# HanielUlises/GCN-GrabCut

Measured on AMD Instinct MI355X. Metric: images/sec end-to-end mask (DUTS-shape batch), higher is better.
Workload: dtype f32

## Files before the change

### gcn-grabcut_amd/csrc/ggc_ccl.h

```cpp
#pragma once
#include <hip/hip_runtime.h>
#include <cstdint>

namespace ggc {

__device__ __forceinline__ int ccl_find(const int32_t* parent, int i) {
    int p = __hip_atomic_load(&parent[i], __ATOMIC_RELAXED, __HIP_MEMORY_SCOPE_AGENT);
    while (p != i) { i = p; p = __hip_atomic_load(&parent[i], __ATOMIC_RELAXED, __HIP_MEMORY_SCOPE_AGENT); }
    return i;
}
__device__ __forceinline__ void ccl_union(int32_t* parent, int a, int b) {
    for (;;) {
        a = ccl_find(parent, a); b = ccl_find(parent, b);
        if (a == b) return;
        if (a < b) { const int t = a; a = b; b = t; }
        const int old = atomicMin(&parent[a], b);
        if (old == a) return;
        a = old;
    }
}

__host__ __device__ inline int ccl_run_start_lane(unsigned long long starts, int lane) {
    const unsigned long long below = starts & ((2ull << lane) - 1ull);
#if defined(__HIP_DEVICE_COMPILE__)
    return 63 - __clzll((long long)below);
#else
    return 63 - __builtin_clzll(below);
#endif
}
__host__ __device__ inline int ccl_run_length(unsigned long long starts, unsigned long long vmask, int lane) {
    const unsigned long long stop = (starts | ~vmask) >> lane >> 1;
#if defined(__HIP_DEVICE_COMPILE__)
    return stop ? __ffsll((long long)stop) : 64 - lane;
#else
    return stop ? __builtin_ffsll((long long)stop) : 64 - lane;
#endif
}

__device__ __forceinline__ int ccl_run_first(bool on, bool same_left, int p) {
    const int lane = threadIdx.x & 63;
    const unsigned long long starts = __ballot(on && (!same_left || lane == 0));
    return p - (lane - ccl_run_start_lane(starts, lane));
}

template <int CONN, class Joined>
__device__ __forceinline__ void ccl_merge_pixel(int32_t* par, int p, int x, bool has_up, int W, size_t flat, Joined joined) {
    static_assert(CONN == 4 || CONN == 8, "4 or 8 neighbours");
    const bool left = x > 0 && joined(p - 1);
    if (left && (flat & 63) == 0) ccl_union(par, p, p - 1);
    if (!has_up) return;
    if constexpr (CONN == 4) {
        if (joined(p - W) && !(left && joined(p - W - 1))) ccl_union(par, p, p - W);
    } else {
        const bool up = joined(p - W);
        const bool ul = x > 0 && joined(p - W - 1), ur = x + 1 < W && joined(p - W + 1);
        if (left) {
            if (ur && !up) ccl_union(par, p, p - W + 1);
        } else if (up) {
            ccl_union(par, p, p - W);
        } else {
            if (ul) ccl_union(par, p, p - W - 1);
            if (ur) ccl_union(par, p, p - W + 1);
        }
    }
}

__device__ __forceinline__ int ccl_compress(int32_t* par, int p) { const int r = ccl_find(par, p); par[p] = r; return r; }
__device__ __forceinline__ void ccl_count_runs(bool valid, bool same_left, unsigned long long vmask, int32_t* counts, size_t cell) {
    const int lane = threadIdx.x & 63;
    const unsigned long long starts = __ballot(valid && (!same_left || lane == 0));
    if (valid && ((starts >> lane) & 1ull)) atomicAdd(&counts[cell], ccl_run_length(starts, vmask, lane));
}

__host__ __device__ inline unsigned long long ccl_best_key(int area, int root) {
    return ((unsigned long long)(unsigned)area << 32) | (unsigned long long)(0xFFFFFFFFu - (unsigned)root);
}
__host__ __device__ inline int ccl_best_root(unsigned long long key) { return (int)(0xFFFFFFFFu - (unsigned)(key & 0xFFFFFFFFull)); }

}
```

### gcn-grabcut_amd/csrc/ggc_context.hip

```cpp
#include "ggc_internal.h"
#include <algorithm>
#include <cstdarg>
#include <cstdlib>
#include <mutex>

static thread_local std::string g_create_err;

namespace ggc {

const Knobs& knobs() {
    static const Knobs k = [] {
        auto num = [](const char* name, int dflt, int lo) { const char* e = std::getenv(name); return e ? std::max(lo, std::atoi(e)) : dflt; };
        Knobs k;
        k.mf_trace = std::getenv("GGC_MF_TRACE") != nullptr;
        k.mf_warm = num("GGC_MF_WARM", 1, 0);
        k.mf_async_push_active = num("GGC_MF_ASYNC_PUSH_ACTIVE", 10000, 0);
        k.mf_async_tile = num("GGC_MF_ASYNC_TILE", 8, 8);
        k.mf_async_hops = num("GGC_MF_ASYNC_HOPS", 24, 1);
        k.mf_async_sweeps = num("GGC_MF_ASYNC_SWEEPS", 12, 1);
        k.mf_dense_launches = num("GGC_MF_DENSE_LAUNCHES", 12, 1);
        k.mf_dense_launches0 = num("GGC_MF_DENSE_LAUNCHES0", 8, 1);
        k.mf_dense_sweeps = num("GGC_MF_DENSE_SWEEPS", 8, 1);
        k.mf_relax_dense = num("GGC_MF_RELAX_DENSE", 3, 1);
        k.mf_partial_rounds = std::min(64, num("GGC_MF_PARTIAL_ROUNDS", 3, 0));
        k.agg_direct = num("GGC_AGG_DIRECT", 0, 0);
        k.slic_seq_connectivity = num("GGC_SLIC_SEQ_CONNECTIVITY", 0, 0);
        k.matte_eval_levels = num("GGC_MATTE_EVAL_LEVELS", 0, 0);
        if (k.matte_eval_levels > 10 || (k.matte_eval_levels && 10 % k.matte_eval_levels != 0)) k.matte_eval_levels = 0;
        k.graph_onchip = num("GGC_GRAPH_ONCHIP", 1, 0);
        k.graph_bands = num("GGC_GRAPH_BANDS", 0, 0);
        if (k.graph_bands > 8) k.graph_bands = 0;
        k.wand_seeds_per_pass = num("GGC_WAND_SEEDS_PER_PASS", 0, 0);
        if (k.wand_seeds_per_pass > 4096) k.wand_seeds_per_pass = 0;
        return k;
    }();
    return k;
}

int set_err(ggc_ctx* ctx, int code, const char* fmt, ...) {
    char buf[1024];
    va_list ap;
    va_start(ap, fmt);
    vsnprintf(buf, sizeof(buf), fmt, ap);
    va_end(ap);
    if (ctx) ctx->err = buf; else g_create_err = buf;
    return code;
}

void* scratch(ggc_ctx* ctx, int slot, size_t bytes) {
    Buf& b = ctx->slots[slot];
    if (bytes == 0) bytes = 16;
    if (b.bytes >= bytes) return b.p;
    if (b.p) {
        if (hipFree(b.p) != hipSuccess) { set_err(ctx, GGC_E_DEVICE, "hipFree failed"); return nullptr; }
        b.p = nullptr; b.bytes = 0;
    }
    size_t want = bytes + bytes / 4;
    want = (want + 255) & ~size_t(255);
    void* p = nullptr;
    if (hipMalloc(&p, want) != hipSuccess) {
        set_err(ctx, GGC_E_OOM, "hipMalloc(%zu) failed for scratch slot %d", want, slot);
        return nullptr;
    }
    b.p = p; b.bytes = want;
    return p;
}

int read_i32(ggc_ctx* ctx, hipStream_t st, const int32_t* dev, int n, std::vector<int32_t>& host) {
    host.resize(n);
    if (ctx->h_pinned && n <= ggc_ctx::H_PINNED_INTS) {
        GGC_HIP(ctx, hipMemcpyAsync(ctx->h_pinned, dev, sizeof(int32_t) * n, hipMemcpyDeviceToHost, st));
        GGC_HIP(ctx, hipStreamSynchronize(st));
        std::copy(ctx->h_pinned, ctx->h_pinned + n, host.begin());
        return GGC_OK;
    }
    GGC_HIP(ctx, hipMemcpyAsync(host.data(), dev, sizeof(int32_t) * n, hipMemcpyDeviceToHost, st));
    GGC_HIP(ctx, hipStreamSynchronize(st));
    return GGC_OK;
}

int check_offsets(ggc_ctx* ctx, const int32_t* off, int n, const char* name, const char* unit, int min_step) {
    GGC_REQUIRE(ctx, off[0] == 0, GGC_E_INVALID_ARG, "%s[0] = %d, expected 0", name, off[0]);
    for (int i = 0; i < n; ++i)
        GGC_REQUIRE(ctx, (int64_t)off[i + 1] - off[i] >= min_step, GGC_E_INVALID_ARG,
                    "%s decreases at %s %d, or steps by less than %d (%d -> %d)", name, unit, i, min_step, off[i], off[i + 1]);
    return GGC_OK;
}

int read_offsets(ggc_ctx* ctx, hipStream_t st, const int32_t* dev, int n, const char* name, const char* unit, int min_step,
                 std::vector<int32_t>& host) {
    const int rc = read_i32(ctx, st, dev, n + 1, host);
    return rc ? rc : check_offsets(ctx, host.data(), n, name, unit, min_step);
}

}

extern "C" {

int ggc_version(void) { return GGC_VERSION; }

int ggc_ctx_create(int device_id, ggc_ctx** out) {
    if (!out) return ggc::set_err(nullptr, GGC_E_INVALID_ARG, "out is NULL");
    *out = nullptr;
    int n = 0;
    hipError_t e = hipGetDeviceCount(&n);
    if (e != hipSuccess || n <= 0)
        return ggc::set_err(nullptr, GGC_E_DEVICE, "no HIP device available (%s)",
                            e == hipSuccess ? "count=0" : hipGetErrorString(e));
    if (device_id < 0 || device_id >= n)
// ... 78 lines not shown
```

### gcn-grabcut_amd/csrc/ggc_internal.h

```cpp
#pragma once
#include <hip/hip_runtime.h>
#include <cstdint>
#include <cstdio>
#include <atomic>
#include <cstring>
#include <map>
#include <string>
#include <type_traits>
#include <vector>
#include "../../include/ggc.h"
#include "../../include/ggc_fmath.h"

namespace ggc {

constexpr int WAVE = 64;

enum Slot : int {
    S_CSR_ROWPTR = 0, S_CSR_COL, S_CSR_EID, S_CSR_CURSOR, S_CSR_SCAN, S_DIS, S_BATCH, S_AGG_PACK,
    S_STATES, S_GATE, S_XW, S_AGG, S_SCORE, S_GVEC, S_HJK,
    S_PRE_A, S_PRE_B, S_PRE_C, S_PRE_D,
    S_SLIC_IMG, S_SLIC_TMP, S_SLIC_CENTERS, S_SLIC_DIST, S_SLIC_LABELS, S_SLIC_AUX,
    S_SLIC_AUX2, S_SLIC_AUX3, S_SLIC_AUX4, S_SLIC_MINMAX,
    S_G_STATS, S_G_FEAT, S_G_PAIRS, S_G_PAIRCNT, S_G_NL, S_G_LISTS, S_G_EDGE_DST,
    S_G_EDGE_ATTR, S_G_PTR, S_G_PRIOR, S_G_AUX, S_G_AUX2, S_G_AUX3, S_G_X,
// ... 1 lines not shown
    S_GC_A, S_GC_B, S_GC_C, S_GC_D, S_GC_E, S_GC_F, S_GC_G, S_GC_H, S_GC_I, S_GC_J,
    S_GC_K, S_GC_L, S_GC_M,
    S_CC_A, S_CC_B, S_CC_C,
    S_MISC_A, S_MISC_B,
    S_CLICK,
    S_MATTE, S_MATTE_MEAN, S_CFMATTE,
    S_FOREGROUND, S_FOREGROUND_VEC,
    S_MATTE_EVAL,
    S_FULLCUT,
    S_GEODESIC,
    S_STROKES,
    S_POLYGONS,
    S_SCISSORS,
    S_OUTLINE, S_OUTLINE_LIST,
    S_DIST, S_DIST_TMP,
    S_WAND,
    S_COUNT
};

struct Buf {
    void*  p = nullptr;
    size_t bytes = 0;
};

struct WeightSet {
    int D = 0;
    int Dt = 0;
    int n_layers = 0;
    int Q = 0, C = 0;
    int heads = 0;
    std::map<std::string, std::vector<float>> host;
    std::map<std::string, Buf> dev;
    bool dev_ok = false;
};

struct GraphState {
    int B = 0, H = 0, W = 0;
    int64_t n_total = 0, e_total = 0;
    std::vector<int64_t> node_ptr, edge_ptr;
    std::vector<int64_t> pair_ptr;
    int64_t max_pairs = 0;
    int n_max = 0;
    const int32_t* n_nodes_dev = nullptr;
    bool valid = false;
};

}

namespace ggc {
struct ProfRec { const char* name; hipEvent_t a, b; };
}

struct ggc_ctx {
    int device = 0;
    std::string err;
    int prof_on = 0;
    double prof_overhead_ms = 0.0;
    std::vector<ggc::ProfRec> prof;
    std::vector<hipEvent_t> prof_pool;
    ggc::Buf slots[ggc::S_COUNT];
    ggc::WeightSet resgcn, gcnnet, gat;
    ggc::GraphState graph;
    int n_cu = 256;
    float prior_two_ce2 = (float)(2 * 0.45 * 0.45), prior_two_cs2 = (float)(2 * 0.40 * 0.40);
    int32_t* h_pinned = nullptr;
    static constexpr int H_PINNED_INTS = 4096;
};

namespace ggc {

struct Knobs {
    int mf_trace;
    int mf_warm;
    int mf_async_push_active;
    int mf_async_tile;
    int mf_async_hops;
    int mf_async_sweeps;
    int mf_dense_launches0, mf_dense_launches;
    int mf_dense_sweeps;
    int mf_relax_dense;
    int mf_partial_rounds;
    int agg_direct;
    int slic_seq_connectivity;
    int matte_eval_levels;
    int graph_onchip;
    int graph_bands;
    int wand_seeds_per_pass;
};
const Knobs& knobs();

int set_err(ggc_ctx* ctx, int code, const char* fmt, ...);
int read_i32(ggc_ctx* ctx, hipStream_t st, const int32_t* dev, int n, std::vector<int32_t>& host);
int read_offsets(ggc_ctx* ctx, hipStream_t st, const int32_t* dev, int n, const char* name, const char* unit, int min_step,
                 std::vector<int32_t>& host);
int check_offsets(ggc_ctx* ctx, const int32_t* off, int n, const char* name, const char* unit, int min_step);
void* scratch(ggc_ctx* ctx, int slot, size_t bytes);
int build_csr(ggc_ctx* ctx, hipStream_t st, int N, int E, const int32_t* src, const int32_t* dst,
              int32_t* row_ptr, int32_t* col, int32_t* eid, int32_t* cursor, float* dis);

#define GGC_HIP(ctx, expr)                                                          \
    do {                                                                            \
        hipError_t _e = (expr);                                                     \
        if (_e != hipSuccess)                                                       \
            return ggc::set_err((ctx), GGC_E_DEVICE, "%s failed: %s (%s:%d)", #expr, \
                                hipGetErrorString(_e), __FILE__, __LINE__);          \
    } while (0)

#define GGC_LAUNCH_CHECK(ctx)                                                        \
    do {                                                                            \
        hipError_t _e = hipGetLastError();                                          \
        if (_e != hipSuccess)                                                       \
            return ggc::set_err((ctx), GGC_E_DEVICE, "kernel launch failed: %s (%s:%d)", \
                                hipGetErrorString(_e), __FILE__, __LINE__);          \
    } while (0)

#define GGC_REQUIRE(ctx, cond, code, ...)                      \
    do {                                                       \
        if (!(cond)) return ggc::set_err((ctx), (code), __VA_ARGS__); \
    } while (0)

template <typename T>
inline T* scratch_t(ggc_ctx* ctx, int slot, size_t count) {
    return reinterpret_cast<T*>(scratch(ctx, slot, count * sizeof(T)));
}

struct Carve {
    char* base = nullptr;
    size_t bytes = 0;
    template <typename T> T* take(size_t count) {
        T* p = base ? reinterpret_cast<T*>(base + bytes) : nullptr;
        bytes += (count * sizeof(T) + 255) & ~size_t(255);
        return p;
    }
};
template <typename Layout>
inline size_t carve_scratch(ggc_ctx* ctx, int slot, Layout&& layout) {
    Carve c;
    layout(c);
    c.base = static_cast<char*>(scratch(ctx, slot, c.bytes));
    if (!c.base) return 0;
    c.bytes = 0;
    layout(c);
    return c.bytes;
}

inline int cdiv(int64_t a, int64_t b) { return (int)((a + b - 1) / b); }

template <int... Ws, typename F>
bool with_width(int D, int& rc, F&& f) {
    return ((D == Ws && (rc = f(std::integral_constant<int, Ws>{}), true)) || ...);
}

struct DeviceOnce {
    std::atomic<unsigned long long> mask{0};
    bool need(int dev) const { return dev < 0 || dev >= 64 || !((mask.load(std::memory_order_acquire) >> dev) & 1ull); }
    void done(int dev) { if (dev >= 0 && dev < 64) mask.fetch_or(1ull << dev, std::memory_order_release); }
};

struct ProfScope {
    ggc_ctx* ctx; hipStream_t st; hipEvent_t b = nullptr;
    ProfScope(ggc_ctx* c, hipStream_t s, const char* name) : ctx(c), st(s) {
        if (!c->prof_on || (c->prof_on == 2 && std::strcmp(name, "gcn_aggregate") != 0)) return;
        hipEvent_t ev[2];
        for (int i = 0; i < 2; ++i) {
            if (!c->prof_pool.empty()) { ev[i] = c->prof_pool.back(); c->prof_pool.pop_back(); }
            else if (hipEventCreate(&ev[i]) != hipSuccess) return;
// ... 67 lines not shown
```

### gcn-grabcut_amd/csrc/ggc_slic.hip

```cpp
#include "ggc_internal.h"
#include "ggc_ccl.h"
#include "ggc_math.h"
#include <cmath>
#include <vector>

namespace ggc {

__global__ void k_minmax_init(int B, uint32_t* mm) {
    const int i = blockIdx.x * blockDim.x + threadIdx.x;
    if (i < B) { mm[2 * i] = 0xFFFFFFFFu; mm[2 * i + 1] = 0u; }
}

__global__ void __launch_bounds__(256) k_minmax(size_t n, const float* __restrict__ img, uint32_t* mm) {
    const float* im = img + (size_t)blockIdx.y * n;
    float lo = INFINITY, hi = -INFINITY;
    for (size_t i = (size_t)blockIdx.x * blockDim.x + threadIdx.x; i < n; i += (size_t)gridDim.x * blockDim.x) {
        const float v = im[i];
        lo = fminf(lo, v); hi = fmaxf(hi, v);
    }
    for (int o = 32; o > 0; o >>= 1) { lo = fminf(lo, __shfl_xor(lo, o, 64)); hi = fmaxf(hi, __shfl_xor(hi, o, 64)); }
    __shared__ float s_lo[4], s_hi[4];
    if ((threadIdx.x & 63) == 0) { s_lo[threadIdx.x >> 6] = lo; s_hi[threadIdx.x >> 6] = hi; }
    __syncthreads();
    if (threadIdx.x == 0) {
// ... 423 lines not shown
        same_left = (p % d.W) > 0 && pending[i - 1] && raw[i - 1] == raw[i];
        r = ccl_compress(parent + base, p);
    }
    ccl_count_runs(valid, same_left, __ballot(valid), csize, base + r);
}

__global__ void __launch_bounds__(256) k_cn_settle(CnDims d, uint8_t* __restrict__ pending, const int32_t* __restrict__ parent,
                                                   const int32_t* __restrict__ csize, int32_t* __restrict__ n_big) {
    const size_t i = (size_t)blockIdx.x * blockDim.x + threadIdx.x;
    if (i >= (size_t)d.B * d.P || !pending[i]) return;
    const size_t base = (i / d.P) * d.P;
    const int p = (int)(i - base), r = parent[i];
    if (csize[base + r] < d.max_size) pending[i] = 0;
    else if (p == r) atomicAdd(n_big, 1);
}

__global__ void __launch_bounds__(64) k_cn_carve(CnDims d, int tag, uint8_t* __restrict__ pending, const int32_t* __restrict__ parent,
                                                 int32_t* __restrict__ csize, int32_t* __restrict__ mark,
                                                 int32_t* __restrict__ queue, int32_t* __restrict__ qtop) {
    const size_t i = (size_t)blockIdx.x * blockDim.x + threadIdx.x;
    if (i >= (size_t)d.B * d.P) return;
    const int b = (int)(i / d.P);
    const size_t base = (size_t)b * d.P;
    const int r = (int)(i - base);
    if (!pending[i] || parent[i] != r || csize[i] < d.max_size) return;
    int32_t* q = queue + base + atomicAdd(&qtop[b], d.max_size);
    int size = 1, visited = 0;
    q[0] = r; mark[base + r] = tag;
    while (visited < size && size < d.max_size) {
        const int pc = q[visited];
        const int yc = pc / d.W, xc = pc - yc * d.W;
#pragma unroll
        for (int k = 0; k < 4; ++k) {
            const int xx = xc + (k == 0 ? 1 : k == 1 ? -1 : 0), yy = yc + (k == 2 ? 1 : k == 3 ? -1 : 0);
            if (xx < 0 || xx >= d.W || yy < 0 || yy >= d.H) continue;
            const int pp = yy * d.W + xx;
            if (pending[base + pp] && parent[base + pp] == r && mark[base + pp] != tag) {
                mark[base + pp] = tag;
                q[size++] = pp;
                if (size >= d.max_size) break;
            }
        }
        visited += 1;
    }
    for (int k = 0; k < size; ++k) pending[base + q[k]] = 0;
    csize[i] = size;
}

__global__ void __launch_bounds__(256) k_cn_kept(CnDims d, const int32_t* __restrict__ parent, const int32_t* __restrict__ csize,
                                                 int32_t* __restrict__ rank) {
    const size_t i = (size_t)blockIdx.x * blockDim.x + threadIdx.x;
    if (i >= (size_t)d.B * d.P) return;
    rank[i] = (parent[i] == (int)(i % d.P) && csize[i] >= d.min_size) ? 1 : 0;
}

__global__ void __launch_bounds__(1024) k_cn_scan(CnDims d, int32_t* __restrict__ rank, int32_t* __restrict__ n_nodes) {
    __shared__ int32_t wsum[16];
    __shared__ int32_t s_carry;
    const int b = blockIdx.x, tid = threadIdx.x, lane = tid & 63, wave = tid >> 6;
    int32_t* a = rank + (size_t)b * d.P;
    if (tid == 0) s_carry = 0;
    __syncthreads();
    for (int base = 0; base < d.P; base += 4096) {
        const int i0 = base + tid * 4;
        int32_t c[4], s = 0;
#pragma unroll
        for (int j = 0; j < 4; ++j) { c[j] = i0 + j < d.P ? a[i0 + j] : 0; s += c[j]; }
        int32_t incl = s;
        for (int o = 1; o < 64; o <<= 1) { const int32_t v = __shfl_up(incl, o, 64); if (lane >= o) incl += v; }
        if (lane == 63) wsum[wave] = incl;
        __syncthreads();
        int32_t run = s_carry + (incl - s), total = 0;
#pragma unroll
        for (int w = 0; w < 16; ++w) { if (w < wave) run += wsum[w]; total += wsum[w]; }
#pragma unroll
        for (int j = 0; j < 4; ++j) { if (i0 + j < d.P) a[i0 + j] = run; run += c[j]; }
        __syncthreads();
        if (tid == 0) s_carry += total;
        __syncthreads();
    }
    if (tid == 0) n_nodes[b] = s_carry > 0 ? s_carry : 1;
}

__global__ void __launch_bounds__(64) k_cn_small(CnDims d, int tag, const int32_t* __restrict__ parent,
                                                 const int32_t* __restrict__ csize, int32_t* __restrict__ mark,
                                                 int32_t* __restrict__ queue, int32_t* __restrict__ qtop,
                                                 int32_t* __restrict__ tgt) {
    const size_t i = (size_t)blockIdx.x * blockDim.x + threadIdx.x;
    if (i >= (size_t)d.B * d.P) return;
    const int b = (int)(i / d.P);
    const size_t base = (size_t)b * d.P;
    const int r = (int)(i - base);
    if (parent[i] != r || csize[i] >= d.min_size) return;
    const int n = csize[i];
    int32_t* q = queue + base + atomicAdd(&qtop[b], n);
    int size = 1, visited = 0, last = -1;
    q[0] = r; mark[base + r] = tag;
    while (visited < size) {
        const int pc = q[visited];
        const int yc = pc / d.W, xc = pc - yc * d.W;
#pragma unroll
        for (int k = 0; k < 4; ++k) {
            const int xx = xc + (k == 0 ? 1 : k == 1 ? -1 : 0), yy = yc + (k == 2 ? 1 : k == 3 ? -1 : 0);
            if (xx < 0 || xx >= d.W || yy < 0 || yy >= d.H) continue;
            const int pp = yy * d.W + xx;
            const int rp = parent[base + pp];
            if (rp == r) { if (mark[base + pp] != tag && size < n) { mark[base + pp] = tag; q[size++] = pp; } }
            else if (rp < r) last = rp;
        }
        visited += 1;
    }
    tgt[i] = last;
}

__global__ void __launch_bounds__(256) k_cn_write(CnDims d, const int32_t* __restrict__ parent, const int32_t* __restrict__ csize,
                                                  const int32_t* __restrict__ rank, const int32_t* __restrict__ tgt,
                                                  int32_t* __restrict__ out) {
    const size_t i = (size_t)blockIdx.x * blockDim.x + threadIdx.x;
    if (i >= (size_t)d.B * d.P) return;
    const size_t base = (i / d.P) * d.P;
    int r = parent[i];
    int lab = 0;
    for (;;) {
        if (csize[base + r] >= d.min_size) { lab = rank[base + r]; break; }
        const int t = tgt[base + r];
        if (t < 0) { lab = 0; break; }
        r = t;
    }
    out[i] = lab;
}


static double np_pairwise_sum(const double* a, int n) {
    if (n < 8) { double s = 0.0; for (int i = 0; i < n; ++i) s += a[i]; return s; }
    double r[8];
    for (int j = 0; j < 8; ++j) r[j] = a[j];
    int i;
    for (i = 8; i < n - (n % 8); i += 8) for (int j = 0; j < 8; ++j) r[j] += a[i + j];
    double res = ((r[0] + r[1]) + (r[2] + r[3])) + ((r[4] + r[5]) + (r[6] + r[7]));
    for (; i < n; ++i) res += a[i];
    return res;
}

struct Grid { int step_y, step_x, start_y, start_x, ny, nx, K; };
static Grid regular_grid(int H, int W, int n_points) {
    Grid g{};
    const double dims[3] = {1.0, (double)(H <= W ? H : W), (double)(H <= W ? W : H)};
    const double space = 1.0 * H * W;
    if (space <= (double)n_points) { g = {1, 1, 0, 0, H, W, H * W}; return g; }
    double st[3];
    for (int i = 0; i < 3; ++i) st[i] = std::pow(space / n_points, 1.0 / 3.0);
    if (dims[0] < st[0] || dims[1] < st[1] || dims[2] < st[2]) {
        for (int dim = 0; dim < 3; ++dim) {
            st[dim] = dims[dim];
            double sp = 1.0;
            for (int j = dim + 1; j < 3; ++j) sp *= dims[j];
            for (int j = dim + 1; j < 3; ++j) st[j] = std::pow(sp / n_points, 1.0 / (3 - dim - 1));
            if (dims[0] >= st[0] && dims[1] >= st[1] && dims[2] >= st[2]) break;
        }
    }
    int starts[3], steps[3];
    for (int i = 0; i < 3; ++i) { starts[i] = (int)std::floor(st[i] / 2.0); steps[i] = (int)std::rint(st[i]); }
    const int iy = (H <= W) ? 1 : 2, ix = (H <= W) ? 2 : 1;
    g.step_y = steps[iy]; g.start_y = starts[iy];
    g.step_x = steps[ix]; g.start_x = starts[ix];
    g.ny = std::max(0, (H - g.start_y + g.step_y - 1) / g.step_y);
    g.nx = std::max(0, (W - g.start_x + g.step_x - 1) / g.step_x);
    g.K = g.ny * g.nx;
    return g;
}

}

using namespace ggc;

static int enforce_connectivity(ggc_ctx* ctx, hipStream_t st, int B, int H, int W, const int32_t* raw, int min_size,
                                int max_size, int32_t* segments, int32_t* n_nodes) {
    const size_t P = (size_t)H * W;
    if (knobs().slic_seq_connectivity) {
        int32_t* queue = scratch_t<int32_t>(ctx, S_SLIC_AUX3, (size_t)B * (size_t)std::max(max_size, 1));
        if (!queue) return GGC_E_OOM;
        GGC_HIP(ctx, hipMemsetAsync(segments, 0xFF, sizeof(int32_t) * (size_t)B * P, st));
        ProfScope prof(ctx, st, "slic_connectivity");
        hipLaunchKernelGGL(k_connectivity_seq, dim3(B), dim3(64), 0, st, H, W, raw, min_size, max_size, queue, segments,
                           n_nodes);
        GGC_LAUNCH_CHECK(ctx);
        return GGC_OK;
    }
    {
        ProfScope prof(ctx, st, "slic_connectivity");
        const size_t BP = (size_t)B * P;
        const CnDims cd{B, H, W, (int)P, min_size, std::max(max_size, 1)};
        int32_t* work = scratch_t<int32_t>(ctx, S_SLIC_AUX3, BP * 6 + (size_t)B * (size_t)cd.max_size + 2 * (size_t)B + 16);
        uint8_t* pending = scratch_t<uint8_t>(ctx, S_SLIC_AUX4, BP);
        if (!work || !pending) return GGC_E_OOM;
        int32_t *parent = work, *csize = work + BP, *rank = work + 2 * BP, *tgt = work + 3 * BP, *mark = work + 4 * BP;
        int32_t* queue = work + 5 * BP;
        int32_t* qtop = work + 6 * BP + (size_t)B * cd.max_size;
        int32_t* n_big = qtop + B;
        GGC_HIP(ctx, hipMemsetAsync(pending, 1, BP, st));
        GGC_HIP(ctx, hipMemsetAsync(mark, 0, sizeof(int32_t) * BP, st));
        const dim3 g1(cdiv(BP, 256)), g2(cdiv(W, 64), cdiv(H, 4), B), g64(cdiv(BP, 64));
        for (int round = 0; round < 4096; ++round) {
            GGC_HIP(ctx, hipMemsetAsync(qtop, 0, sizeof(int32_t) * (B + 1), st));
            hipLaunchKernelGGL(k_cn_reset, g1, dim3(256), 0, st, cd, raw, pending, parent, csize);
            hipLaunchKernelGGL(k_cn_merge, g2, dim3(256), 0, st, cd, raw, pending, parent);
            hipLaunchKernelGGL(k_cn_size, g1, dim3(256), 0, st, cd, raw, pending, parent, csize);
            hipLaunchKernelGGL(k_cn_settle, g1, dim3(256), 0, st, cd, pending, parent, csize, n_big);
            GGC_LAUNCH_CHECK(ctx);
            int32_t h_big = 0;
            GGC_HIP(ctx, hipMemcpyAsync(&h_big, n_big, sizeof(int32_t), hipMemcpyDeviceToHost, st));
            GGC_HIP(ctx, hipStreamSynchronize(st));
            if (h_big == 0) break;
            hipLaunchKernelGGL(k_cn_carve, g64, dim3(64), 0, st, cd, round + 1, pending, parent, csize, mark, queue, qtop);
            GGC_LAUNCH_CHECK(ctx);
        }
        hipLaunchKernelGGL(k_cn_kept, g1, dim3(256), 0, st, cd, parent, csize, rank);
        hipLaunchKernelGGL(k_cn_scan, dim3(B), dim3(1024), 0, st, cd, rank, n_nodes);
        GGC_HIP(ctx, hipMemsetAsync(qtop, 0, sizeof(int32_t) * (B + 1), st));
        hipLaunchKernelGGL(k_cn_small, g64, dim3(64), 0, st, cd, 0x7FFFFFFF, parent, csize, mark, queue, qtop, tgt);
        hipLaunchKernelGGL(k_cn_write, g1, dim3(256), 0, st, cd, parent, csize, rank, tgt, segments);
        GGC_LAUNCH_CHECK(ctx);
    }
    return GGC_OK;
}

extern "C" int ggc_slic(ggc_ctx* ctx, ggc_stream stream, int B, int H, int W, const float* image,
                        int n_segments, float compactness, float sigma, int rescale_input,
                        int32_t* segments, int32_t* n_nodes) {
    if (!ctx) return GGC_E_INVALID_ARG;
    GGC_REQUIRE(ctx, B >= 1 && H >= 1 && W >= 1 && B <= 65535, GGC_E_SHAPE, "bad shape B=%d H=%d W=%d", B, H, W);
    GGC_REQUIRE(ctx, image && segments && n_nodes, GGC_E_INVALID_ARG, "null pointer");
    GGC_REQUIRE(ctx, n_segments >= 1 && compactness > 0.0f && sigma >= 0.0f, GGC_E_INVALID_ARG,
                "bad SLIC parameters n_segments=%d compactness=%g sigma=%g", n_segments, compactness, sigma);
    GGC_REQUIRE(ctx, (size_t)H * W < (1u << 30), GGC_E_SHAPE, "image too large");
    GGC_HIP(ctx, hipSetDevice(ctx->device));
    hipStream_t st = reinterpret_cast<hipStream_t>(stream);
    const size_t P = (size_t)H * W;

    const Grid seed = regular_grid(H, W, n_segments);
    GGC_REQUIRE(ctx, seed.K >= 1, GGC_E_SHAPE, "no SLIC seeds for %dx%d with n_segments=%d", H, W, n_segments);
    const Grid win = regular_grid(H, W, seed.K);
    SlicGeom g{};
    g.H = H; g.W = W; g.K = seed.K;
    g.ny = seed.ny; g.nx = seed.nx; g.start_y = seed.start_y; g.start_x = seed.start_x;
    g.step_y = seed.step_y; g.step_x = seed.step_x;
    g.win_y = win.step_y; g.win_x = win.step_x;
    const float step = (float)std::max(std::max(seed.step_y, seed.step_x), 1);
    g.sw = (float)(1.0 / (double)(step * step));

    float* img_a = scratch_t<float>(ctx, S_SLIC_IMG, (size_t)B * P * 3);
    float* img_b = scratch_t<float>(ctx, S_SLIC_TMP, (size_t)B * P * 3);
    uint32_t* mm = scratch_t<uint32_t>(ctx, S_SLIC_MINMAX, (size_t)B * 2);
    float* centers = scratch_t<float>(ctx, S_SLIC_CENTERS, (size_t)B * g.K * 5);
    int4* bounds = scratch_t<int4>(ctx, S_SLIC_AUX, (size_t)B * g.K);
    int32_t* raw = scratch_t<int32_t>(ctx, S_SLIC_LABELS, (size_t)B * P);
    int32_t* stale = scratch_t<int32_t>(ctx, S_SLIC_AUX2, (size_t)B * 10);
    if (!img_a || !img_b || !mm || !centers || !bounds || !raw || !stale) return GGC_E_OOM;

    hipLaunchKernelGGL(k_minmax_init, dim3(cdiv(B, 256)), dim3(256), 0, st, B, mm);
    hipLaunchKernelGGL(k_minmax, dim3(std::min(cdiv(P * 3, 256 * 8), 48), B), dim3(256), 0, st, P * 3, image, mm);
    hipLaunchKernelGGL(k_lab2, dim3(cdiv(P, 256), B), dim3(256), 0, st, P, image, mm, rescale_input, img_a);
    GGC_LAUNCH_CHECK(ctx);
    const float ratio = (float)(1.0 / (double)compactness);
    const float* km_img = nullptr;
    if (sigma > 0.0f) {
        GaussW gw{};
        gw.r = (int)(4.0 * (double)sigma + 0.5);
        GGC_REQUIRE(ctx, gw.r <= MAX_RADIUS, GGC_E_UNSUPPORTED, "sigma=%g needs radius %d > %d", sigma, gw.r, MAX_RADIUS);
        ggc_gaussian_taps((double)sigma, gw.r, gw.w);
        const double sum = np_pairwise_sum(gw.w, 2 * gw.r + 1);
        for (int i = 0; i < 2 * gw.r + 1; ++i) gw.w[i] = gw.w[i] / sum;
        GGC_REQUIRE(ctx, H <= 65535, GGC_E_SHAPE, "H=%d exceeds the launch grid", H);
        const dim3 grid(cdiv((size_t)W * 3, 256), H, B);
        if (gw.r == 4) {
            hipLaunchKernelGGL((k_gauss_v<4>), dim3(cdiv((size_t)W * 3, 256), cdiv(H, GV_ROWS), B), dim3(256), 0, st, H, W, img_a, gw, img_b);
            hipLaunchKernelGGL((k_gauss<1, 4>), grid, dim3(256), 0, st, H, W, img_b, gw, ratio, 1, img_a);
        } else {
            hipLaunchKernelGGL((k_gauss<0, 0>), grid, dim3(256), 0, st, H, W, img_a, gw, 1.0f, 0, img_b);
            hipLaunchKernelGGL((k_gauss<1, 0>), grid, dim3(256), 0, st, H, W, img_b, gw, ratio, 1, img_a);
        }
        km_img = img_a;
    } else {
        hipLaunchKernelGGL(k_scale, dim3(cdiv((size_t)B * P * 3, 256)), dim3(256), 0, st, (size_t)B * P * 3, img_a,
                           ratio, img_b);
        km_img = img_b;
    }
    GGC_LAUNCH_CHECK(ctx);
    hipLaunchKernelGGL(k_init_centers, dim3(cdiv(g.K, 256), B), dim3(256), 0, st, g, centers, bounds);
    GGC_HIP(ctx, hipMemsetAsync(raw, 0, sizeof(int32_t) * (size_t)B * P, st));
    GGC_HIP(ctx, hipMemsetAsync(stale, 0, sizeof(int32_t) * (size_t)B * 10, st));
    for (int it = 0; it < 10; ++it) {
        {
            ProfScope prof(ctx, st, "slic_assign");
            hipLaunchKernelGGL(k_slic_assign, dim3(cdiv(W, TILE_W), cdiv(H, TILE_H), B), dim3(256), 0, st, g, km_img,
                               centers, bounds, raw, stale + (size_t)it * B);
        }
        if (it < 9) {
            ProfScope prof(ctx, st, "slic_update");
            hipLaunchKernelGGL(k_slic_update, dim3(cdiv(g.K, 4 * UPD_GROUPS), B), dim3(256), 0, st, g, km_img, raw,
                               stale + (size_t)it * B, centers, bounds);
        }
        GGC_LAUNCH_CHECK(ctx);
    }
    const double seg_size = (double)P / (double)g.K;
    const int min_size = (int)(0.5 * seg_size), max_size = (int)(3.0 * seg_size);
    return enforce_connectivity(ctx, st, B, H, W, raw, min_size, max_size, segments, n_nodes);
// ... 289 lines not shown
```

Before: 3890.

## Add tiled LDS connected-components path for SLIC connectivity enforcement

Adds a new SLIC connectivity path, on by default, that labels components inside 64x16 tiles using union-find in shared memory. A separate pass then merges the tile borders in global memory. Small components are reassigned by a per-component BFS kernel with LDS queues, and labels come from per-row bitmask popcounts plus a prefix scan. This replaces the multi-round reset/merge/size/settle loop and its per-round host sync in the common case. If any component reaches max_size it falls back to the old rounds path, which wastes the tile work in that case.

```diff
diff --git a/gcn-grabcut_amd/csrc/ggc_ccl.h b/gcn-grabcut_amd/csrc/ggc_ccl.h
--- a/gcn-grabcut_amd/csrc/ggc_ccl.h
+++ b/gcn-grabcut_amd/csrc/ggc_ccl.h
@@ -18,6 +18,31 @@
         if (old == a) return;
         a = old;
     }
+}
+
+__device__ __forceinline__ int ccl_find_lds(const int* par, int i) {
+    int p = __hip_atomic_load(&par[i], __ATOMIC_RELAXED, __HIP_MEMORY_SCOPE_WORKGROUP);
+    while (p != i) { i = p; p = __hip_atomic_load(&par[i], __ATOMIC_RELAXED, __HIP_MEMORY_SCOPE_WORKGROUP); }
+    return i;
+}
+__device__ __forceinline__ void ccl_union_lds(int* par, int a, int b) {
+    for (;;) {
+        a = ccl_find_lds(par, a); b = ccl_find_lds(par, b);
+        if (a == b) return;
+        if (a < b) { const int t = a; a = b; b = t; }
+        const int old = atomicMin(&par[a], b);
+        if (old == a) return;
+        a = old;
+    }
+}
+
+__host__ __device__ inline int ccl_rank_in_word(unsigned long long word, int lane) {
+    const unsigned long long below = word & ((1ull << lane) - 1ull);
+#if defined(__HIP_DEVICE_COMPILE__)
+    return __popcll(below);
+#else
+    return __builtin_popcountll(below);
+#endif
 }
 
 __host__ __device__ inline int ccl_run_start_lane(unsigned long long starts, int lane) {
diff --git a/gcn-grabcut_amd/csrc/ggc_context.hip b/gcn-grabcut_amd/csrc/ggc_context.hip
--- a/gcn-grabcut_amd/csrc/ggc_context.hip
+++ b/gcn-grabcut_amd/csrc/ggc_context.hip
@@ -25,6 +25,7 @@
         k.mf_partial_rounds = std::min(64, num("GGC_MF_PARTIAL_ROUNDS", 3, 0));
         k.agg_direct = num("GGC_AGG_DIRECT", 0, 0);
         k.slic_seq_connectivity = num("GGC_SLIC_SEQ_CONNECTIVITY", 0, 0);
+        k.slic_cn_tiles = num("GGC_SLIC_CN_TILES", 1, 0);
         k.matte_eval_levels = num("GGC_MATTE_EVAL_LEVELS", 0, 0);
         if (k.matte_eval_levels > 10 || (k.matte_eval_levels && 10 % k.matte_eval_levels != 0)) k.matte_eval_levels = 0;
         k.graph_onchip = num("GGC_GRAPH_ONCHIP", 1, 0);
diff --git a/gcn-grabcut_amd/csrc/ggc_internal.h b/gcn-grabcut_amd/csrc/ggc_internal.h
--- a/gcn-grabcut_amd/csrc/ggc_internal.h
+++ b/gcn-grabcut_amd/csrc/ggc_internal.h
@@ -107,6 +107,7 @@
     int mf_partial_rounds;
     int agg_direct;
     int slic_seq_connectivity;
+    int slic_cn_tiles;
     int matte_eval_levels;
     int graph_onchip;
     int graph_bands;
diff --git a/gcn-grabcut_amd/csrc/ggc_slic.hip b/gcn-grabcut_amd/csrc/ggc_slic.hip
--- a/gcn-grabcut_amd/csrc/ggc_slic.hip
+++ b/gcn-grabcut_amd/csrc/ggc_slic.hip
@@ -529,7 +529,7 @@
     if (tid == 0) n_nodes[b] = s_carry > 0 ? s_carry : 1;
 }
 
-__global__ void __launch_bounds__(64) k_cn_small(CnDims d, int tag, const int32_t* __restrict__ parent,
+__global__ void __launch_bounds__(64) k_cn_small(CnDims d, int tag, int min_n, const int32_t* __restrict__ parent,
                                                  const int32_t* __restrict__ csize, int32_t* __restrict__ mark,
                                                  int32_t* __restrict__ queue, int32_t* __restrict__ qtop,
                                                  int32_t* __restrict__ tgt) {
@@ -538,7 +538,7 @@
     const int b = (int)(i / d.P);
     const size_t base = (size_t)b * d.P;
     const int r = (int)(i - base);
-    if (parent[i] != r || csize[i] >= d.min_size) return;
+    if (parent[i] != r || csize[i] >= d.min_size || csize[i] < min_n) return;
     const int n = csize[i];
     int32_t* q = queue + base + atomicAdd(&qtop[b], n);
     int size = 1, visited = 0, last = -1;
@@ -572,6 +572,236 @@
         if (csize[base + r] >= d.min_size) { lab = rank[base + r]; break; }
         const int t = tgt[base + r];
         if (t < 0) { lab = 0; break; }
+        r = t;
+    }
+    out[i] = lab;
+}
+
+constexpr int CN_TW = 64, CN_TH = 16;
+constexpr int CN_QCAP = 256;
+constexpr int CN_SEEN_ROW = 2 * CN_QCAP / 32;
+static_assert(CN_TW == 64 && CN_TH % 4 == 0, "a tile row is one wave, the rows split over four waves");
+typedef unsigned long long cn_word;
+
+__global__ void __launch_bounds__(256) k_cn_tile(CnDims d, const int32_t* __restrict__ raw, int32_t* __restrict__ parent,
+                                                 int32_t* __restrict__ csize, cn_word* __restrict__ troot) {
+    constexpr int RPW = CN_TH / 4;
+    __shared__ int s_lab[CN_TH * CN_TW], s_par[CN_TH * CN_TW], s_cnt[CN_TH * CN_TW];
+    const int lane = threadIdx.x & 63, wave = threadIdx.x >> 6;
+    const int x = blockIdx.x * CN_TW + lane, y0 = blockIdx.y * CN_TH;
+    const size_t base = (size_t)blockIdx.z * d.P;
+    int lab[RPW], root[RPW];
+    bool on[RPW], same_left[RPW];
+#pragma unroll
+    for (int j = 0; j < RPW; ++j) {
+        const int ty = wave * RPW + j, t = ty * CN_TW + lane;
+        on[j] = x < d.W && y0 + ty < d.H;
+        lab[j] = on[j] ? raw[base + (size_t)(y0 + ty) * d.W + x] : 0;
+        const int left = __shfl_up(lab[j], 1, 64);
+        same_left[j] = on[j] && lane > 0 && left == lab[j];
+        const int first = ccl_run_first(on[j], same_left[j], t);
+        s_lab[t] = lab[j];
+        s_par[t] = on[j] ? first : t;
+        s_cnt[t] = 0;
+    }
+    __syncthreads();
+#pragma unroll
+    for (int j = 0; j < RPW; ++j) {
+        const int ty = wave * RPW + j, t = ty * CN_TW + lane;
+        if (on[j] && ty > 0 && s_lab[t - CN_TW] == lab[j] && !(same_left[j] && s_lab[t - CN_TW - 1] == lab[j]))
+            ccl_union_lds(s_par, t, t - CN_TW);
+    }
+    __syncthreads();
+#pragma unroll
+    for (int j = 0; j < RPW; ++j) {
+        const int ty = wave * RPW + j, t = ty * CN_TW + lane;
+        root[j] = on[j] ? ccl_find_lds(s_par, t) : t;
+        const cn_word vmask = __ballot(on[j]);
+        const cn_word starts = __ballot(on[j] && (!same_left[j] || lane == 0));
+        if (on[j] && ((starts >> lane) & 1ull)) atomicAdd(&s_cnt[root[j]], ccl_run_length(starts, vmask, lane));
+    }
+    __syncthreads();
+#pragma unroll
+    for (int j = 0; j < RPW; ++j) {
+        const int ty = wave * RPW + j, t = ty * CN_TW + lane, y = y0 + ty;
+        const bool is_root = on[j] && root[j] == t;
+        const cn_word roots = __ballot(is_root);
+        if (y >= d.H) continue;
+        if (lane == 0) troot[((size_t)blockIdx.z * d.H + y) * gridDim.x + blockIdx.x] = roots;
+        if (!on[j]) continue;
+        const size_t p = base + (size_t)y * d.W + x;
+        parent[p] = (y0 + root[j] / CN_TW) * d.W + blockIdx.x * CN_TW + root[j] % CN_TW;
+        if (is_root) csize[p] = s_cnt[t];
+    }
+}
+
+__global__ void __launch_bounds__(256) k_cn_border(CnDims d, const int32_t* __restrict__ raw, int32_t* __restrict__ parent) {
+    const int nvb = (d.W - 1) / CN_TW, nhb = (d.H - 1) / CN_TH;
+    const int idx = blockIdx.x * blockDim.x + threadIdx.x;
+    if (idx >= nvb * d.H + nhb * d.W) return;
+    const size_t base = (size_t)blockIdx.y * d.P;
+    const int32_t* r = raw + base;
+    int32_t* par = parent + base;
+    if (idx < nvb * d.H) {
+        const int x = (idx / d.H + 1) * CN_TW, y = idx % d.H, p = y * d.W + x;
+        if (r[p] != r[p - 1]) return;
+        if (y % CN_TH != 0 && r[p - d.W] == r[p] && r[p - d.W - 1] == r[p]) return;
+        ccl_union(par, p, p - 1);
+    } else {
+        const int j = idx - nvb * d.H;
+        const int y = (j / d.W + 1) * CN_TH, x = j % d.W, p = y * d.W + x;
+        if (r[p] != r[p - d.W]) return;
+        if (x % CN_TW != 0 && r[p - 1] == r[p] && r[p - d.W - 1] == r[p]) return;
+        ccl_union(par, p, p - d.W);
+    }
+}
+
+__global__ void __launch_bounds__(256) k_cn_finish(CnDims d, int32_t* __restrict__ parent, int32_t* __restrict__ csize,
+                                                   const cn_word* __restrict__ troot) {
+    const int lane = threadIdx.x & 63, x = blockIdx.x * CN_TW + lane, y = blockIdx.y * 4 + (threadIdx.x >> 6);
+    if (x >= d.W || y >= d.H) return;
+    const size_t base = (size_t)blockIdx.z * d.P;
+    int32_t* par = parent + base;
+    const int p = y * d.W + x;
+    const int p0 = __hip_atomic_load(&par[p], __ATOMIC_RELAXED, __HIP_MEMORY_SCOPE_AGENT);
+    if (p0 == p) return;
+    const int r = ccl_find(par, p0);
+    if (r != p0) par[p] = r;
+    if ((troot[((size_t)blockIdx.z * d.H + y) * gridDim.x + blockIdx.x] >> lane) & 1ull) atomicAdd(&csize[base + r], csize[base + p]);
+}
+
+__global__ void __launch_bounds__(256) k_cn_flag(CnDims d, const int32_t* __restrict__ parent, const int32_t* __restrict__ csize,
+                                                 cn_word* __restrict__ kmask, int32_t* __restrict__ counters,
+                                                 int32_t* __restrict__ lcount, int32_t* __restrict__ list) {
+    const int lane = threadIdx.x & 63, x = blockIdx.x * CN_TW + lane, y = blockIdx.y * 4 + (threadIdx.x >> 6);
+    if (y >= d.H) return;
+    const size_t i = (size_t)blockIdx.z * d.P + (size_t)y * d.W + x;
+    const bool root = x < d.W && parent[i] == y * d.W + x;
+    const int n = root ? csize[i] : 0;
+    const bool small = root && n < d.min_size, fits = small && n <= CN_QCAP;
+    const cn_word kept = __ballot(root && n >= d.min_size), big = __ballot(root && n >= d.max_size);
+    const cn_word listed = __ballot(fits), spilled = __ballot(small && !fits);
+    if (lane == 0) {
+        kmask[((size_t)blockIdx.z * d.H + y) * gridDim.x + blockIdx.x] = kept;
+        if (big) atomicAdd(&counters[0], __popcll(big));
+        if (spilled) atomicAdd(&counters[2], __popcll(spilled));
+    }
+    if (!listed) return;
+    int pos = 0;
+    if (lane == 0) pos = atomicAdd(&lcount[blockIdx.z], __popcll(listed));
+    pos = __shfl(pos, 0, 64);
+    if (fits) list[(size_t)blockIdx.z * d.P + pos + ccl_rank_in_word(listed, lane)] = y * d.W + x;
+}
+
+__global__ void __launch_bounds__(256) k_cn_rank(int n_seg, const cn_word* __restrict__ kmask, int32_t* __restrict__ prefix,
+                                                 int32_t* __restrict__ n_nodes, const int32_t* __restrict__ lcount,
+                                                 int32_t* __restrict__ counters) {
+    __shared__ int32_t wsum[4];
+    const int tid = threadIdx.x, lane = tid & 63, wave = tid >> 6;
+    const size_t off = (size_t)blockIdx.x * n_seg;
+    int32_t carry = 0;
+    for (int s0 = 0; s0 < n_seg; s0 += 256) {
+        const int s = s0 + tid;
+        const int32_t c = s < n_seg ? __popcll(kmask[off + s]) : 0;
+        int32_t incl = c;
+        for (int o = 1; o < 64; o <<= 1) { const int32_t v = __shfl_up(incl, o, 64); if (lane >= o) incl += v; }
+        if (lane == 63) wsum[wave] = incl;
+        __syncthreads();
+        int32_t run = carry + incl - c, total = 0;
+#pragma unroll
+        for (int w = 0; w < 4; ++w) { if (w < wave) run += wsum[w]; total += wsum[w]; }
+        if (s < n_seg) prefix[off + s] = run;
+        carry += total;
+        __syncthreads();
+    }
+    if (tid == 0) {
+        n_nodes[blockIdx.x] = carry > 0 ? carry : 1;
+        if (lcount[blockIdx.x] > 0) atomicMax(&counters[1], lcount[blockIdx.x]);
+    }
+}
+
+__global__ void __launch_bounds__(64) k_cn_replay(CnDims d, const int32_t* __restrict__ parent, const int32_t* __restrict__ csize,
+                                                  const int32_t* __restrict__ list, const int32_t* __restrict__ lcount,
+                                                  int32_t* __restrict__ tgt) {
+    __shared__ int s_q[CN_QCAP];
+    __shared__ unsigned s_seen[CN_QCAP * CN_SEEN_ROW];
+    const int lane = threadIdx.x;
+    if ((int)blockIdx.x >= lcount[blockIdx.y]) return;
+    const size_t base = (size_t)blockIdx.y * d.P;
+    const int32_t* par = parent + base;
+    const int r = list[base + blockIdx.x], yr = r / d.W, xr = r - yr * d.W;
+    const size_t i = base + r;
+    const int n = min(csize[i], CN_QCAP);
+    for (int k = lane; k < n * CN_SEEN_ROW; k += 64) s_seen[k] = 0;
+    __syncthreads();
+    if (lane == 0) { s_q[0] = r; s_seen[CN_QCAP >> 5] = 1u << (CN_QCAP & 31); }
+    __syncthreads();
+    int head = 0, size = 1, last = -1;
+    while (head < size) {
+        const int cnt = min(64, size - head);
+        const bool active = lane < cnt;
+        const int pc = active ? s_q[head + lane] : 0;
+        const int yc = pc / d.W, xc = pc - yc * d.W;
+        int pp[4], rp[4], word[4];
+        unsigned bit[4];
+        bool inb[4];
+#pragma unroll
+        for (int k = 0; k < 4; ++k) {
+            const int xx = xc + (k == 0 ? 1 : k == 1 ? -1 : 0), yy = yc + (k == 2 ? 1 : k == 3 ? -1 : 0);
+            inb[k] = active && xx >= 0 && xx < d.W && yy >= 0 && yy < d.H;
+            pp[k] = yy * d.W + xx;
+            rp[k] = inb[k] ? par[pp[k]] : 0x7FFFFFFF;
+            const int dy = yy - yr, col = xx - xr + CN_QCAP;
+            const bool in_map = dy >= 0 && dy < n && col >= 0 && col < 2 * CN_QCAP;
+            word[k] = in_map ? dy * CN_SEEN_ROW + (col >> 5) : -1;
+            bit[k] = 1u << (col & 31);
+        }
+        int mine = -1;
+        unsigned m = 0;
+#pragma unroll
+        for (int k = 0; k < 4; ++k) {
+            if (rp[k] == r) { if (word[k] >= 0 && !(s_seen[word[k]] & bit[k])) m |= 1u << k; }
+            else if (rp[k] < r) mine = rp[k];
+        }
+        const cn_word have = __ballot(mine >= 0);
+        if (have) last = __shfl(mine, 63 - __clzll((long long)have), 64);
+        for (;;) {
+            const cn_word todo = __ballot(m != 0);
+            if (!todo || size >= n) break;
+            const int src = __ffsll((long long)todo) - 1;
+            const int k0 = __ffs((int)m) - 1;
+            const int c = __shfl(k0 == 0 ? pp[0] : k0 == 1 ? pp[1] : k0 == 2 ? pp[2] : pp[3], src, 64);
+            const int cw = __shfl(k0 == 0 ? word[0] : k0 == 1 ? word[1] : k0 == 2 ? word[2] : word[3], src, 64);
+            const unsigned cb = __shfl(k0 == 0 ? bit[0] : k0 == 1 ? bit[1] : k0 == 2 ? bit[2] : bit[3], src, 64);
+            if (lane == 0) { s_q[size] = c; s_seen[cw] |= cb; }
+            size += 1;
+#pragma unroll
+            for (int k = 0; k < 4; ++k) if (pp[k] == c) m &= ~(1u << k);
+        }
+        head += cnt;
+        __syncthreads();
+    }
+    if (lane == 0) tgt[i] = last;
+}
+
+__global__ void __launch_bounds__(256) k_cn_label(CnDims d, int n_tx, const int32_t* __restrict__ parent,
+                                                  const int32_t* __restrict__ csize, const int32_t* __restrict__ tgt,
+                                                  const cn_word* __restrict__ kmask, const int32_t* __restrict__ prefix,
+                                                  int32_t* __restrict__ out) {
+    const size_t i = (size_t)blockIdx.x * blockDim.x + threadIdx.x;
+    if (i >= (size_t)d.B * d.P) return;
+    const size_t b = i / d.P, base = b * d.P;
+    int r = parent[i];
+    int lab = 0;
+    for (;;) {
+        if (csize[base + r] >= d.min_size) {
+            const int yr = r / d.W, xr = r - yr * d.W;
+            const size_t s = (b * d.H + yr) * n_tx + xr / CN_TW;
+            lab = prefix[s] + ccl_rank_in_word(kmask[s], xr % CN_TW);
+            break;
+        }
+        const int t = tgt[base + r];
+        if (t < 0) break;
         r = t;
     }
     out[i] = lab;
@@ -621,6 +851,92 @@
 
 using namespace ggc;
 
+static int connectivity_rounds(ggc_ctx* ctx, hipStream_t st, const CnDims& cd, const int32_t* raw, int32_t* segments,
+                               int32_t* n_nodes) {
+    ProfScope prof(ctx, st, "slic_cn_rounds");
+    const int B = cd.B, H = cd.H, W = cd.W;
+    const size_t BP = (size_t)B * cd.P;
+    int32_t* work = scratch_t<int32_t>(ctx, S_SLIC_AUX3, BP * 6 + (size_t)B * (size_t)cd.max_size + 2 * (size_t)B + 16);
+    uint8_t* pending = scratch_t<uint8_t>(ctx, S_SLIC_AUX4, BP);
+    if (!work || !pending) return GGC_E_OOM;
+    int32_t *parent = work, *csize = work + BP, *rank = work + 2 * BP, *tgt = work + 3 * BP, *mark = work + 4 * BP;
+    int32_t* queue = work + 5 * BP;
+    int32_t* qtop = work + 6 * BP + (size_t)B * cd.max_size;
+    int32_t* n_big = qtop + B;
+    GGC_HIP(ctx, hipMemsetAsync(pending, 1, BP, st));
+    GGC_HIP(ctx, hipMemsetAsync(mark, 0, sizeof(int32_t) * BP, st));
+    const dim3 g1(cdiv(BP, 256)), g2(cdiv(W, 64), cdiv(H, 4), B), g64(cdiv(BP, 64));
+    for (int round = 0; round < 4096; ++round) {
+        GGC_HIP(ctx, hipMemsetAsync(qtop, 0, sizeof(int32_t) * (B + 1), st));
+        hipLaunchKernelGGL(k_cn_reset, g1, dim3(256), 0, st, cd, raw, pending, parent, csize);
+        hipLaunchKernelGGL(k_cn_merge, g2, dim3(256), 0, st, cd, raw, pending, parent);
+        hipLaunchKernelGGL(k_cn_size, g1, dim3(256), 0, st, cd, raw, pending, parent, csize);
+        hipLaunchKernelGGL(k_cn_settle, g1, dim3(256), 0, st, cd, pending, parent, csize, n_big);
+        GGC_LAUNCH_CHECK(ctx);
+        int32_t h_big = 0;
+        GGC_HIP(ctx, hipMemcpyAsync(&h_big, n_big, sizeof(int32_t), hipMemcpyDeviceToHost, st));
+        GGC_HIP(ctx, hipStreamSynchronize(st));
+        if (h_big == 0) break;
+        hipLaunchKernelGGL(k_cn_carve, g64, dim3(64), 0, st, cd, round + 1, pending, parent, csize, mark, queue, qtop);
+        GGC_LAUNCH_CHECK(ctx);
+    }
+    hipLaunchKernelGGL(k_cn_kept, g1, dim3(256), 0, st, cd, parent, csize, rank);
+    hipLaunchKernelGGL(k_cn_scan, dim3(B), dim3(1024), 0, st, cd, rank, n_nodes);
+    GGC_HIP(ctx, hipMemsetAsync(qtop, 0, sizeof(int32_t) * (B + 1), st));
+    hipLaunchKernelGGL(k_cn_small, g64, dim3(64), 0, st, cd, 0x7FFFFFFF, 0, parent, csize, mark, queue, qtop, tgt);
+    hipLaunchKernelGGL(k_cn_write, g1, dim3(256), 0, st, cd, parent, csize, rank, tgt, segments);
+    GGC_LAUNCH_CHECK(ctx);
+    return GGC_OK;
+}
+
+static int connectivity_tiles(ggc_ctx* ctx, hipStream_t st, const CnDims& cd, const int32_t* raw, int32_t* segments,
+                              int32_t* n_nodes, bool& done) {
+    const int B = cd.B, H = cd.H, W = cd.W, n_tx = cdiv(W, CN_TW), n_seg = H * n_tx;
+    const size_t BP = (size_t)B * cd.P, n_words = (size_t)B * n_seg;
+    const bool may_spill = cd.min_size - 1 > CN_QCAP;
+    int32_t *parent, *csize, *tgt, *list, *prefix, *counters, *lcount, *mark = nullptr, *queue = nullptr, *qtop = nullptr;
+    cn_word *troot, *kmask;
+    if (!carve_scratch(ctx, S_SLIC_AUX3, [&](Carve& c) {
+            parent = c.take<int32_t>(BP); csize = c.take<int32_t>(BP); tgt = c.take<int32_t>(BP); list = c.take<int32_t>(BP);
+            troot = c.take<cn_word>(n_words); kmask = c.take<cn_word>(n_words); prefix = c.take<int32_t>(n_words);
+            counters = c.take<int32_t>(4 + (size_t)B); lcount = counters + 4;
+            if (may_spill) { mark = c.take<int32_t>(BP); queue = c.take<int32_t>(BP); qtop = c.take<int32_t>((size_t)B + 1); }
+        }))
+        return GGC_E_OOM;
+    const dim3 g_tile(n_tx, cdiv(H, CN_TH), B), g_row(n_tx, cdiv(H, 4), B);
+    const int n_border = ((W - 1) / CN_TW) * H + ((H - 1) / CN_TH) * W;
+    std::vector<int32_t> h;
+    {
+        ProfScope tiles(ctx, st, "slic_cn_tiles");
+        GGC_HIP(ctx, hipMemsetAsync(counters, 0, sizeof(int32_t) * (4 + (size_t)B), st));
+        hipLaunchKernelGGL(k_cn_tile, g_tile, dim3(256), 0, st, cd, raw, parent, csize, troot);
+        if (n_border > 0) hipLaunchKernelGGL(k_cn_border, dim3(cdiv(n_border, 256), B), dim3(256), 0, st, cd, raw, parent);
+        hipLaunchKernelGGL(k_cn_finish, g_row, dim3(256), 0, st, cd, parent, csize, troot);
+        hipLaunchKernelGGL(k_cn_flag, g_row, dim3(256), 0, st, cd, parent, csize, kmask, counters, lcount, list);
+        hipLaunchKernelGGL(k_cn_rank, dim3(B), dim3(256), 0, st, n_seg, kmask, prefix, n_nodes, lcount, counters);
+        GGC_LAUNCH_CHECK(ctx);
+        const int rc = read_i32(ctx, st, counters, 3, h);
+        if (rc != GGC_OK) return rc;
+    }
+    if (h[0] > 0) return GGC_OK;
+    if (h[1] > 0) {
+        ProfScope replay(ctx, st, "slic_cn_replay");
+        hipLaunchKernelGGL(k_cn_replay, dim3(h[1], B), dim3(64), 0, st, cd, parent, csize, list, lcount, tgt);
+    }
+    if (h[2] > 0) {
+        ProfScope spill(ctx, st, "slic_cn_spill");
+        GGC_REQUIRE(ctx, may_spill, GGC_E_DEVICE, "SLIC connectivity: %d small components above the queue capacity", h[2]);
+        GGC_HIP(ctx, hipMemsetAsync(mark, 0, sizeof(int32_t) * BP, st));
+        GGC_HIP(ctx, hipMemsetAsync(qtop, 0, sizeof(int32_t) * ((size_t)B + 1), st));
+        hipLaunchKernelGGL(k_cn_small, dim3(cdiv(BP, 64)), dim3(64), 0, st, cd, 0x7FFFFFFF, CN_QCAP + 1, parent, csize, mark,
+                           queue, qtop, tgt);
+    }
+    hipLaunchKernelGGL(k_cn_label, dim3(cdiv(BP, 256)), dim3(256), 0, st, cd, n_tx, parent, csize, tgt, kmask, prefix, segments);
+    GGC_LAUNCH_CHECK(ctx);
+    done = true;
+    return GGC_OK;
+}
+
 static int enforce_connectivity(ggc_ctx* ctx, hipStream_t st, int B, int H, int W, const int32_t* raw, int min_size,
                                 int max_size, int32_t* segments, int32_t* n_nodes) {
     const size_t P = (size_t)H * W;
@@ -634,42 +950,15 @@
         GGC_LAUNCH_CHECK(ctx);
         return GGC_OK;
     }
-    {
-        ProfScope prof(ctx, st, "slic_connectivity");
-        const size_t BP = (size_t)B * P;
-        const CnDims cd{B, H, W, (int)P, min_size, std::max(max_size, 1)};
-        int32_t* work = scratch_t<int32_t>(ctx, S_SLIC_AUX3, BP * 6 + (size_t)B * (size_t)cd.max_size + 2 * (size_t)B + 16);
-        uint8_t* pending = scratch_t<uint8_t>(ctx, S_SLIC_AUX4, BP);
-        if (!work || !pending) return GGC_E_OOM;
-        int32_t *parent = work, *csize = work + BP, *rank = work + 2 * BP, *tgt = work + 3 * BP, *mark = work + 4 * BP;
-        int32_t* queue = work + 5 * BP;
-        int32_t* qtop = work + 6 * BP + (size_t)B * cd.max_size;
-        int32_t* n_big = qtop + B;
-        GGC_HIP(ctx, hipMemsetAsync(pending, 1, BP, st));
-        GGC_HIP(ctx, hipMemsetAsync(mark, 0, sizeof(int32_t) * BP, st));
-        const dim3 g1(cdiv(BP, 256)), g2(cdiv(W, 64), cdiv(H, 4), B), g64(cdiv(BP, 64));
-        for (int round = 0; round < 4096; ++round) {
-            GGC_HIP(ctx, hipMemsetAsync(qtop, 0, sizeof(int32_t) * (B + 1), st));
-            hipLaunchKernelGGL(k_cn_reset, g1, dim3(256), 0, st, cd, raw, pending, parent, csize);
-            hipLaunchKernelGGL(k_cn_merge, g2, dim3(256), 0, st, cd, raw, pending, parent);
-            hipLaunchKernelGGL(k_cn_size, g1, dim3(256), 0, st, cd, raw, pending, parent, csize);
-            hipLaunchKernelGGL(k_cn_settle, g1, dim3(256), 0, st, cd, pending, parent, csize, n_big);
-            GGC_LAUNCH_CHECK(ctx);
-            int32_t h_big = 0;
-            GGC_HIP(ctx, hipMemcpyAsync(&h_big, n_big, sizeof(int32_t), hipMemcpyDeviceToHost, st));
-            GGC_HIP(ctx, hipStreamSynchronize(st));
-            if (h_big == 0) break;
-            hipLaunchKernelGGL(k_cn_carve, g64, dim3(64), 0, st, cd, round + 1, pending, parent, csize, mark, queue, qtop);
-            GGC_LAUNCH_CHECK(ctx);
-        }
-        hipLaunchKernelGGL(k_cn_kept, g1, dim3(256), 0, st, cd, parent, csize, rank);
-        hipLaunchKernelGGL(k_cn_scan, dim3(B), dim3(1024), 0, st, cd, rank, n_nodes);
-        GGC_HIP(ctx, hipMemsetAsync(qtop, 0, sizeof(int32_t) * (B + 1), st));
-        hipLaunchKernelGGL(k_cn_small, g64, dim3(64), 0, st, cd, 0x7FFFFFFF, parent, csize, mark, queue, qtop, tgt);
-        hipLaunchKernelGGL(k_cn_write, g1, dim3(256), 0, st, cd, parent, csize, rank, tgt, segments);
-        GGC_LAUNCH_CHECK(ctx);
-    }
-    return GGC_OK;
+    ProfScope prof(ctx, st, "slic_connectivity");
+    const size_t BP = (size_t)B * P;
+    const CnDims cd{B, H, W, (int)P, min_size, std::max(max_size, 1)};
+    if (knobs().slic_cn_tiles) {
+        bool done = false;
+        const int rc = connectivity_tiles(ctx, st, cd, raw, segments, n_nodes, done);
+        if (rc != GGC_OK || done) return rc;
+    }
+    return connectivity_rounds(ctx, st, cd, raw, segments, n_nodes);
 }
 
 extern "C" int ggc_slic(ggc_ctx* ctx, ggc_stream stream, int B, int H, int W, const float* image,
```

Result: faster. 3964, median of 6 (+1.9%).
